# Janspiry/Image-Super-Resolution-via-Iterative-Refinement

Measured on NVIDIA H100. Metric: diffusion steps/sec (batch16, 16->128 SR3), higher is better.
Workload: dtype bf16

## Files before the change

image-super-resolution-via-iterative-refinement_b200/csrc/engine.cu:

```cuda
#include <cuda.h>
#include <cuda_runtime.h>

#include <cmath>
#include <cstdarg>
#include <cstdlib>
#include <cstring>
#include <functional>
#include <limits>
#include <map>
#include <memory>
#include <mutex>
#include <stdexcept>
#include <string>
#include <vector>

#include "../../include/sr3_b200.h"
#include "aux_kernels.cuh"
#include "attn_wgmma.cuh"
#include "train_kernels.cuh"

using namespace sr3;
typedef __nv_bfloat16 bf16;

namespace {
// ... 81 lines not shown
    long long b_rows = 0; int b_K = 0;
    std::vector<KSlab> slabs;
    int block_n = 128;
    int w_box = 16, h_box = 8, b_box = 1;
    int mh = 1;
    int pingpong = 0;
    int tall = 0;
    int a_box_w = 0, a_box_h = 0, a_box_b = 0;
    int a_half_off = 0;
    bool b_is_param = false;
    int ksplit_max = 1;
    int tiles_w = 1, tiles_h = 1, tiles_b = 1, n_tiles = 1, nz = 1;
    int a_zstep = 0, b_zrows = 0;
    int z_phase = 0; long long z_off_hi = 0, z_off_lo = 0;
    int passes = 1, lo_b_col = 0, lo_a_chan[2] = {0, 0};
    long long lo_out_off = 0, lo_t_off = 0;
    int mode = 0, OW = 0, OH = 1, OB = 1, n_valid = 0;
    int out_imgs = 0;
    float scale = 1.f;
    const float* bias = nullptr; const float* bias2 = nullptr; int bias2_stride = 0;
    const float* resid = nullptr; OutSpec rs{};
    float* out_f32 = nullptr; OutSpec os{};
    bf16* out_bf16 = nullptr; OutSpec hs{};
    bf16* out_t = nullptr; int t_col0 = 0, t_rows = 0, t_ld = 0, t_per = 1;
    double* stats = nullptr; int stats_C = 0, stats_coff = 0;
    const StepCtl* ctl = nullptr; PostParams post{};
};

OutSpec nhwc_out(int H, int W, int C, long long off = 0) {
    OutSpec s; s.sZ = 0; s.sB = 1LL * H * W * C; s.sH = 1LL * W * C; s.sW = C; s.off = off; return s;
}

constexpr int SMEM_LIMIT = 232448;
int pick_stages(int block_n, int a_stage_bytes, int b_taps, bool resid, int num_k) {
    int s = GEMM_MAX_STAGES;
    if (const char* e = getenv("SR3_STAGES")) s = atoi(e);
    if (s > GEMM_MAX_STAGES) s = GEMM_MAX_STAGES;
    while (s > 1 && gemm_smem_bytes(block_n, a_stage_bytes, b_taps, s, resid, num_k) > SMEM_LIMIT) --s;
    if (s < 1) s = 1;
    return s;
}
int current_device() { int dev = 0; CK(cudaGetDevice(&dev)); return dev; }
int num_sms() {
    static std::map<int, int> cache;
    static std::mutex mu;
    std::lock_guard<std::mutex> lock(mu);
    const int dev = current_device();
    auto it = cache.find(dev);
    if (it != cache.end()) return it->second;
    int n = 0;
    CK(cudaDeviceGetAttribute(&n, cudaDevAttrMultiProcessorCount, dev));
    cache[dev] = n;
    return n;
}
bool first_use_on_device(std::vector<int>& seen) {
    static std::mutex mu;
    std::lock_guard<std::mutex> lock(mu);
    const int dev = current_device();
    for (int d : seen) if (d == dev) return false;
    seen.push_back(dev);
    return true;
}
template <typename... KArgs, typename... Args>
void launch_k(void (*kernel)(KArgs...), dim3 grid, dim3 block, size_t smem, cudaStream_t st, Args&&... args) {
    cudaLaunchConfig_t cfg{};
    cfg.gridDim = grid; cfg.blockDim = block; cfg.dynamicSmemBytes = smem; cfg.stream = st;
    cudaLaunchAttribute attr[1];
    attr[0].id = cudaLaunchAttributeProgrammaticStreamSerialization;
    attr[0].val.programmaticStreamSerializationAllowed = 1;
    cfg.attrs = attr; cfg.numAttrs = 1;
    CK(cudaLaunchKernelEx(&cfg, kernel, std::forward<Args>(args)...));
// ... 197 lines not shown
        if (d.out_f32 && d.resid) REQUIRE(zo == zr, "output and residual must share the batch coordinate");
        if (!d.out_f32) p.out_map = p.res_map;
        if (!d.resid) p.res_map = p.out_map;
        p.epi_c4_is_z = (d.out_f32 ? zo : zr) ? 1 : 0;
    } else {
        p.out_map = p.b_map; p.res_map = p.b_map;
    }
    p.ksplit = 1;
    {
        const int tiles = d.tiles_w * d.tiles_h * d.tiles_b * d.n_tiles * d.nz;
        const int ks = d.ksplit_max;
        if (ks > 1 && !d.pingpong && d.mode == 0 && d.out_f32 && d.block_n >= 32 && d.n_valid % 32 == 0) {
            int want = num_sms() / tiles;
            if (want > ks) want = ks;
            if (want > p.num_k * d.passes / 2) want = p.num_k * d.passes / 2;
            const int units = d.mh * (d.block_n / 32) * 4;
            if (want > units) want = units;
            want = fit_split(want, tiles);
            if (want > 1) {
                p.ksplit = want;
                p.ws = static_cast<float*>(mem.alloc((size_t)tiles * want * d.mh * 128 * d.block_n * sizeof(float), false));
                p.counters = static_cast<unsigned int*>(mem.alloc((size_t)tiles * sizeof(unsigned int)));
            }
        }
    }
    const int total_tiles = d.tiles_w * d.tiles_h * d.tiles_b * d.n_tiles * d.nz * p.ksplit;
    int ctas = total_tiles < num_sms() ? total_tiles : num_sms();
    if (const char* e = getenv("SR3_MAX_CTAS")) { int v = atoi(e); if (v > 0 && v < ctas) ctas = v; }
    REQUIRE(p.ksplit == 1 || ctas == total_tiles, "split-K launch needs one CTA per (tile, split) pair: %d CTAs for %d (SR3_MAX_CTAS with a split tile)", ctas, total_tiles);
    const dim3 grid(ctas, 1, 1);
    const int bn = d.block_n;
    const int mh = d.mh;
    const bool res_smem = p.tma_epi && d.resid != nullptr && p.ksplit <= 1;
    p.stages = pick_stages(d.block_n, p.a_stage_bytes, p.b_taps, res_smem, p.num_k);
    const int smem = gemm_smem_bytes(bn, p.a_stage_bytes, p.b_taps, p.stages, res_smem, p.num_k);
    REQUIRE(smem <= SMEM_LIMIT, "gemm shared memory %d exceeds the limit", smem);
    init_gemm_attrs();
    REQUIRE((bn == 16 || bn == 32 || bn == 64 || bn == 128 || bn == 256) && (mh == 1 || (mh == 2 && bn <= 128 && bn != 32)), "unsupported tile %dx%d", 128 * mh, bn);
    const bool pp = d.pingpong != 0;
    REQUIRE(!pp || (gemm_pingpong_ok(bn, mh) && p.ksplit == 1 && d.mode == 0), "no ping-pong form of tile %dx%d (split %d)", 128 * mh, bn, p.ksplit);
    if (geo) {
        geo->tall = d.tall; geo->mh = mh; geo->block_n = bn; geo->h_box = d.h_box; geo->b_box = d.b_box;
        geo->ksplit = p.ksplit; geo->stages = p.stages; geo->ctas = ctas; geo->tiles = total_tiles / p.ksplit; geo->res_smem = res_smem ? 1 : 0;
    }
    if (schedule) *schedule = pp ? 1 : 0;
    std::shared_ptr<GemmParams> sp = std::make_shared<GemmParams>(p);
    if (g_gemm_registry) {
        GemmHandle h; h.p = sp; h.w_ptr = d.b_ptr; h.w_bytes = 2LL * d.b_rows * d.b_K; h.w_is_param = d.b_is_param; h.bn = bn; h.mh = mh;
        g_gemm_registry->push_back(h);
    }
    return [sp, grid, bn, mh, pp, smem](cudaStream_t st) {
        const GemmParams& p = *sp;
        if (pp) {
            if (mh == 2) launch_gemm_bn<64, 2, true>(p, grid, smem, st);
            else if (bn == 64) launch_gemm_bn<64, 1, true>(p, grid, smem, st);
            else launch_gemm_bn<128, 1, true>(p, grid, smem, st);
            return;
        }
        switch (bn) {
            case 16: if (mh == 2) launch_gemm_bn<16, 2>(p, grid, smem, st); else launch_gemm_bn<16, 1>(p, grid, smem, st); break;
            case 32: launch_gemm_bn<32, 1>(p, grid, smem, st); break;
            case 64: if (mh == 2) launch_gemm_bn<64, 2>(p, grid, smem, st); else launch_gemm_bn<64, 1>(p, grid, smem, st); break;
            case 128: if (mh == 2) launch_gemm_bn<128, 2>(p, grid, smem, st); else launch_gemm_bn<128, 1>(p, grid, smem, st); break;
            default: launch_gemm_bn<256, 1>(p, grid, smem, st); break;
        }
    };
}

// ... 103 lines not shown
                    const double cpp = model(tiles, nstage * npass, stage_bytes, c.mh * 128, c.bn, sp1, true);
                    if (cpp < best_pp) { best_pp = cpp; pp_mh = c.mh; pp_bn = c.bn; }
                }
                if (c.bn == 128 && has_resid && sp <= 1) continue;
                if (cost < best) { best = cost; mh = c.mh; bn = c.bn; split = sp; }
            }
            if (!shape_forced && pp_bn && (pp_force || (pp_auto && best_pp < best))) { mh = pp_mh; bn = pp_bn; split = 1; pp = 1; }
        }
        if (const char* e = getenv("SR3_TALL_BN")) { int v = atoi(e); if ((v == 32 || v == 64 || v == 128) && cout % v == 0) { bn = v; split = 16; } }
        if (const char* e = getenv("SR3_TALL_MH")) { int v = atoi(e); if (v == 1 || v == 2) { mh = v; split = 16; } }
        if (mh == 2 && bn == 32) bn = 64;
        if (shape_forced) pp = (pp_force && gemm_pingpong_ok(bn, mh)) ? 1 : 0;
        if (pp) split = 1;
        d.mh = mh; d.block_n = bn; d.ksplit_max = split; d.pingpong = pp;
        geom(mh, d.h_box, d.b_box);
        d.a_box_w = 8; d.a_box_b = d.b_box;
        if (mh == 2 && d.b_box == 1) { d.a_box_h = 34; d.a_half_off = 16 * 1024; }
        else if (mh == 2) { d.a_box_h = 18; d.a_half_off = 18 * 1024; }
        else { d.a_box_h = 18; d.a_half_off = 0; }
    } else {
        d.tall = 0; d.mh = 1;
        pick_image_box(OW, OH, d.w_box, d.h_box, d.b_box);
        d.block_n = pick_block_n(cout);
        const long long mt = (long long)(OW / d.w_box) * ((OH + d.h_box - 1) / d.h_box) * ((Bt + d.b_box - 1) / d.b_box) * nz;
        if (getenv("SR3_BLOCK_N") == nullptr && cout % 32 == 0) {
            const int nstage = (((int)d.slabs.size() + 2) / 3) * npass;
            double best = 1e300, best_pp = 1e300;
            int pp_bn = 0;
            for (int bn = 128; bn >= 32; bn >>= 1) {
                if (cout % bn != 0) continue;
                int sp = 1;
                const long long tiles = mt * (cout / bn);
                const double cost = model(tiles, nstage, 3ll * (16384 + bn * 128), 128, bn, sp);
                if (gemm_pingpong_ok(bn, 1) && gemm_smem_bytes(bn, 3 * 16384, 3, 2, has_resid, nstage / npass) <= SMEM_LIMIT) {
                    int sp1 = 1;
                    const double cpp = model(tiles, nstage, 3ll * (16384 + bn * 128), 128, bn, sp1, true);
                    if (cpp < best_pp) { best_pp = cpp; pp_bn = bn; }
                }
                if (bn == 128 && sp > 1) continue;
                if (cost < best) { best = cost; d.block_n = bn; d.ksplit_max = sp; }
            }
            if (pp_bn && (pp_force || (pp_auto && best_pp < best))) { d.block_n = pp_bn; d.ksplit_max = 1; d.pingpong = 1; }
        } else if (pp_force && gemm_pingpong_ok(d.block_n, 1)) {
            d.pingpong = 1;
        }
    }
    if (d.pingpong) d.ksplit_max = 1;
    if (const char* e = getenv("SR3_KSPLIT")) d.ksplit_max = atoi(e);
    d.tiles_w = OW / d.w_box; d.tiles_h = (OH + d.h_box - 1) / d.h_box; d.tiles_b = (Bt + d.b_box - 1) / d.b_box;
}

void pick_image_box(int W, int H, int& w_box, int& h_box, int& b_box) {
    w_box = W < 16 ? W : 16;
    h_box = 128 / w_box;
    if (h_box > H) h_box = H;
    if (w_box * h_box < 32) h_box = 32 / w_box;
    b_box = 128 / (w_box * h_box);
}

int pick_block_n(int cout) {
    if (const char* e = getenv("SR3_BLOCK_N")) { int v = atoi(e); if (v == 32 || v == 64 || v == 128 || v == 256) if (cout % v == 0) return v; }
    if (cout % 128 == 0) return 128;
    if (cout % 64 == 0) return 64;
    return 16;
}

void add_conv_slabs(std::vector<KSlab>& slabs, int a_sel, int cin, int ksize, int stride, int b_col0, int row = 0) {
// ... 2034 lines not shown
```

image-super-resolution-via-iterative-refinement_b200/csrc/gemm_wgmma.cuh:

```cuda
#pragma once
#include <cuda.h>
#include <type_traits>
#include "ptx.cuh"

namespace sr3 {

struct OutSpec {
    long long sZ, sB, sH, sW, off;
};

struct StepCtl {
    int t_cur;
    int t_next;
    int nl_from_table;
    int out_mode;
    int use_noise_buf;
    int write_mean;
    int clip;
    int update_state;
    unsigned long long seed;
    unsigned long long sample_offset;
};

struct PostParams {
// ... 18 lines not shown
struct StageDesc {
    int ntaps;
    int a_multi;
    int a_sel;
    int pad0;
    StageTap tap[3];
    int pad1, pad2;
};

struct GemmParams {
    CUtensorMap a_map[2];
    CUtensorMap b_map;
    CUtensorMap out_map;
    CUtensorMap res_map;
    const StageDesc* ktab;
    int num_k;
    int a_stage_bytes;
    int a_box_bytes;
    int a_half_off;
    int b_taps;
    int tiles_w, tiles_h, tiles_b;
    int n_tiles, nz;
    int tma_epi;
    int epi_c4_is_z;
    int ksplit;
    float* ws;
    unsigned int* counters;
    const void* pf_ptr;
    long long pf_bytes;
    int w_box, h_box, b_box;
    int w_shift, h_shift;
    int a_zstep, b_zrows;
    int stages;
    int mode;
    int OW, OH, OB, n_valid;
    float scale;
    const float* bias;
    const float* bias2;
    int bias2_stride;
    const float* resid;
    OutSpec rs;
    float* out_f32;
    OutSpec os;
    __nv_bfloat16* out_bf16;
    OutSpec hs;
    __nv_bfloat16* out_t;
    int t_col0, t_rows, t_ld, t_per;
    double* stats;
    int stats_C, stats_coff;
    const StepCtl* ctl;
    PostParams post;
    int z_phase;
    long long z_off_hi, z_off_lo;
    int passes, lo_b_col, lo_a_chan[2];
    long long lo_out_off, lo_t_off;
};

constexpr int GEMM_THREADS = 288;
constexpr int GEMM_EPI_WARPS = 8;
constexpr int GEMM_PRODUCER_WARP = 8;
constexpr int GEMM_MAX_STAGES = 8;
__host__ __device__ constexpr int gemm_epi_warp_bytes(bool resid) { return resid ? 12288 : 4096; }
__host__ __device__ constexpr int gemm_epi_bytes(bool resid) { return GEMM_EPI_WARPS * gemm_epi_warp_bytes(resid); }
constexpr int GEMM_MAX_K = 160;
constexpr int GEMM_HDR_BYTES = 2048;
__host__ __device__ constexpr bool gemm_single_wg(int block_n, int mh) { return mh == 1 && block_n <= 32; }
__host__ __device__ constexpr bool gemm_pingpong_ok(int block_n, int mh) { return (mh == 2 && block_n == 64) || (mh == 1 && (block_n == 64 || block_n == 128)); }
constexpr int GEMM_ORDER_BAR = 2;
__host__ __device__ constexpr int gemm_stage_readers(int block_n, int mh, bool pp) { return (pp || gemm_single_wg(block_n, mh)) ? 1 : 2; }
__host__ __device__ constexpr int gemm_aux_bytes(int num_k) {
    return GEMM_HDR_BYTES + ((num_k * 96 + 127) / 128) * 128  + GEMM_EPI_WARPS * 2 * 32 * 4 ;
}

__host__ __device__ constexpr int gemm_stage_bytes(int block_n, int a_stage_bytes, int b_taps) { return a_stage_bytes + b_taps * block_n * 128; }
__host__ __device__ constexpr int gemm_smem_bytes(int block_n, int a_stage_bytes, int b_taps, int stages, bool resid, int num_k) {
    return stages * gemm_stage_bytes(block_n, a_stage_bytes, b_taps) + gemm_epi_bytes(resid) + 1024  + gemm_aux_bytes(num_k);
}

__device__ __forceinline__ void philox4x32_10(uint32_t (&c)[4], uint32_t k0, uint32_t k1) {
#pragma unroll
    for (int r = 0; r < 10; ++r) {
        const uint32_t hi0 = __umulhi(0xD2511F53u, c[0]), lo0 = 0xD2511F53u * c[0];
        const uint32_t hi1 = __umulhi(0xCD9E8D57u, c[2]), lo1 = 0xCD9E8D57u * c[2];
        const uint32_t n0 = hi1 ^ c[1] ^ k0, n1 = lo1, n2 = hi0 ^ c[3] ^ k1, n3 = lo0;
        c[0] = n0; c[1] = n1; c[2] = n2; c[3] = n3;
        k0 += 0x9E3779B9u; k1 += 0xBB67AE85u;
    }
}
__device__ __forceinline__ void box_muller(uint32_t a, uint32_t b, float& z0, float& z1) {
    const float u1 = (static_cast<float>(a) + 1.0f) * 2.3283064365386963e-10f;
    const float u2 = static_cast<float>(b) * 2.3283064365386963e-10f;
    const float r = sqrtf(-2.0f * logf(u1));
    float s, c;
    sincospif(2.0f * u2, &s, &c);
    z0 = r * c; z1 = r * s;
}

__device__ __forceinline__ double stats_quantize(double v) { return rint(v * 1048576.0) * (1.0 / 1048576.0); }

__device__ __forceinline__ float warp_column_sums(float (&v)[32]) {
    const uint32_t lane = lane_id();
#pragma unroll
    for (int half = 16; half >= 1; half >>= 1) {
        const bool up = (lane & half) != 0;
#pragma unroll
        for (int j = 0; j < half; ++j) {
            const float keep = up ? v[j + half] : v[j];
            const float send = up ? v[j] : v[j + half];
            v[j] = keep + __shfl_xor_sync(0xffffffffu, send, half);
// ... 23 lines not shown
    if (t > 0) {
        if (ctl.use_noise_buf) {
            for (int c = 0; c < q.C; ++c) z[c] = q.noise_buf[(static_cast<long long>(img) * q.C + c) * plane + pix];
        } else {
            uint32_t ctr[4] = {static_cast<uint32_t>(pix), static_cast<uint32_t>(ctl.sample_offset + img), static_cast<uint32_t>(t),
                               static_cast<uint32_t>((ctl.sample_offset + img) >> 32)};
            philox4x32_10(ctr, static_cast<uint32_t>(ctl.seed), static_cast<uint32_t>(ctl.seed >> 32));
            box_muller(ctr[0], ctr[1], z[0], z[1]);
            box_muller(ctr[2], ctr[3], z[2], z[3]);
        }
    }
    for (int c = 0; c < q.C; ++c) {
        const long long idx = (static_cast<long long>(img) * q.C + c) * plane + pix;
        const float xt = q.x_state[idx];
        float x0 = __fsub_rn(__fmul_rn(c1, xt), __fmul_rn(c2, eps[c]));
        if (ctl.clip) x0 = fminf(fmaxf(x0, -1.0f), 1.0f);
        const float mean = __fadd_rn(__fmul_rn(pc1, x0), __fmul_rn(pc2, xt));
        if (ctl.write_mean) q.mean_out[idx] = mean;
        const float xn = __fadd_rn(mean, __fmul_rn(z[c], sigma));
        if (ctl.update_state) {
            q.x_state[idx] = xn;
            __nv_bfloat16* ib = q.in_buf + (static_cast<long long>(img) * plane + pix) * q.in_C + q.in_coff + c;
            const __nv_bfloat16 hi = __float2bfloat16_rn(xn);
            *ib = hi;
            if (q.in_lo_off) ib[q.in_lo_off] = __float2bfloat16_rn(xn - __bfloat162float(hi));
        }
    }
}

__device__ __forceinline__ void gemm_stage_setup(const GemmParams& p, const GemmParams* pm, const uint32_t base, uint8_t* base_ptr, const int block_n,
                                                 const int mh, const bool pp) {
    const int stages = p.stages;
    const int stage_bytes = p.a_stage_bytes + p.b_taps * block_n * 128;
    const bool use_res_tma = p.tma_epi && p.resid != nullptr && p.ksplit <= 1;
    const int epi_bytes = GEMM_EPI_WARPS * gemm_epi_warp_bytes(use_res_tma);
    uint8_t* aux_ptr = base_ptr + GEMM_HDR_BYTES + stages * stage_bytes + epi_bytes;
    {
        const int4* src = reinterpret_cast<const int4*>(p.ktab);
        int4* dst = reinterpret_cast<int4*>(aux_ptr);
        for (int i = threadIdx.x; i < p.num_k * 6; i += blockDim.x) dst[i] = __ldg(&src[i]);
    }
    if (threadIdx.x == 0) {
        tma_prefetch_desc(&pm->a_map[0]);
        tma_prefetch_desc(&pm->a_map[1]);
        tma_prefetch_desc(&pm->b_map);
        if (p.tma_epi) { tma_prefetch_desc(&pm->out_map); tma_prefetch_desc(&pm->res_map); }
        const uint32_t bar_base = base;
        const uint32_t consumers = gemm_stage_readers(block_n, mh, pp);
        for (int s = 0; s < stages; ++s) {
            mbar_init(bar_base + 8u * s, 1);
            mbar_init(bar_base + 8u * (GEMM_MAX_STAGES + s), consumers);
        }
        for (int w = 0; w < 2 * GEMM_EPI_WARPS; ++w) mbar_init(bar_base + 8u * (2 * GEMM_MAX_STAGES + w), 1);
        fence_mbar_init();
    }
}

template <int WN, int CW, int CL>
__device__ __forceinline__ void acc_chunk_rows(const float (&acc)[2][WN / 2], float* buf, float (&v)[32]) {
    static_assert(CW <= 32 && (CL + 1) * CW <= WN, "accumulator chunk");
    const int lane = static_cast<int>(lane_id());
    __syncwarp();
#pragma unroll
    for (int i = 0; i < 2; ++i) {
#pragma unroll
        for (int j = (CL * CW) / 2; j < ((CL + 1) * CW) / 2; j += 2) {
            const int r = (lane >> 2) + 8 * i + 16 * ((j >> 1) & 1);
            const int cc = 8 * (j >> 2) - CL * CW + 2 * (lane & 3);
            *reinterpret_cast<float2*>(buf + r * 32 + (cc ^ ((r & 7) << 2))) = make_float2(acc[i][j], acc[i][j + 1]);
// ... 36 lines not shown
                }
            }
        }
        clear();
    }
    __device__ __forceinline__ void start(const GemmParams& p, const int im, const int nb0, const int ch0, const int lane) {
        if (im != img || nb0 != n0) { flush(p, ch0, lane); img = im; n0 = nb0; }
    }
    __device__ __forceinline__ void add(const int c, const double s, const double q) {
#pragma unroll
        for (int cc = 0; cc < N; ++cc)
            if (cc == c) { sum[cc] += s; sq[cc] += q; }
    }
};

template <int BLOCK_N, int MH, bool PP = false>
__device__ __forceinline__ void gemm_tile_body(const GemmParams& p, const GemmParams* pm, const uint32_t base, uint8_t* base_ptr,
                                               const int cta, const int ncta) {
    static_assert(!PP || gemm_pingpong_ok(BLOCK_N, MH), "ping-pong tile shape");
    constexpr int B_BYTES = BLOCK_N * 128;
    constexpr bool SINGLE = !PP && gemm_single_wg(BLOCK_N, MH);
    constexpr int WN = (PP || SINGLE || MH == 2) ? BLOCK_N : BLOCK_N / 2;
    constexpr int AH = PP ? MH : 1;
    constexpr int CW = WN < 32 ? WN : 32;
    constexpr int NCH = BLOCK_N >= 32 ? BLOCK_N / 32 : 1;
    constexpr int NITEMS = MH * NCH;
    constexpr int OWN = PP ? NITEMS : SINGLE ? 1 : NITEMS / 2;
    constexpr int NSTAT = PP ? NCH : OWN;
    static_assert(WN % CW == 0 && AH * WN <= 128, "accumulator shape");

    const int stages = p.stages;
    const int stage_bytes = p.a_stage_bytes + p.b_taps * B_BYTES;
    const bool use_res_tma = p.tma_epi && p.resid != nullptr && p.ksplit <= 1;
    const int epi_warp_bytes = gemm_epi_warp_bytes(use_res_tma);
    const int epi_bytes = GEMM_EPI_WARPS * epi_warp_bytes;
    const uint32_t bar_base = base;
    const uint32_t stage_base = base + GEMM_HDR_BYTES;
    uint8_t* stage_ptr = base_ptr + GEMM_HDR_BYTES;
    const uint32_t epi_base = stage_base + stages * stage_bytes;
    auto full_bar = [&](int s) { return bar_base + 8u * s; };
    auto empty_bar = [&](int s) { return bar_base + 8u * (GEMM_MAX_STAGES + s); };
    auto res_bar = [&](int w, int b) { return bar_base + 8u * (2 * GEMM_MAX_STAGES + 2 * w + b); };
    uint8_t* aux_ptr = stage_ptr + stages * stage_bytes + epi_bytes;
    StageDesc* ktab_s = reinterpret_cast<StageDesc*>(aux_ptr);
    float* bias_s = reinterpret_cast<float*>(aux_ptr + ((p.num_k * 96 + 127) / 128) * 128);

    const int warp = threadIdx.x >> 5;
    const int lane = threadIdx.x & 31;
    const int tiles_m = p.tiles_w * p.tiles_h * p.tiles_b;
    const int ksplit = p.ksplit > 1 ? p.ksplit : 1;
    const int total_tiles = tiles_m * p.n_tiles * p.nz * ksplit;
    const int num_kt = p.num_k * (p.passes > 1 ? p.passes : 1);
    gemm_stage_setup(p, pm, base, base_ptr, BLOCK_N, MH, PP);
    __syncthreads();
    if (warp == 2 && lane == 0 && p.pf_bytes > 0) {
        long long chunk = ((p.pf_bytes + ncta - 1) / ncta + 15) & ~15ll;
        const long long off = chunk * cta;
        if (off < p.pf_bytes) {
            if (off + chunk > p.pf_bytes) chunk = (p.pf_bytes - off) & ~15ll;
            const char* src = static_cast<const char*>(p.pf_ptr) + off;
            for (long long done = 0; done < chunk; done += 65536) {
                const unsigned int n = static_cast<unsigned int>(chunk - done < 65536 ? chunk - done : 65536);
                if (n >= 16) asm volatile("cp.async.bulk.prefetch.L2.global [%0], %1;" ::"l"(src + done), "r"(n) : "memory");
            }
        }
    }
    pdl_launch_dependents();
// ... 21 lines not shown
            decode(tile, w0, h0, b0, n0, z);
            const int brow = n0 + z * p.b_zrows;
            const int zdw = p.z_phase ? (z & 1) : 0, zdh = p.z_phase ? (z >> 1) : 0;
            const int sp = tile % ksplit;
            const int k0 = (num_kt * sp) / ksplit, k1 = (num_kt * (sp + 1)) / ksplit;
            for (int k = k0; k < k1; ++k) {
                mbar_wait(empty_bar(s), ph ^ 1u);
                if (elect_one_sync()) {
                    const int pass = k / p.num_k;
                    const StageDesc& e = ktab_s[k - pass * p.num_k];
                    const int a_lo = (pass == 2) ? p.lo_a_chan[e.a_sel] : 0, b_lo = (pass == 1) ? p.lo_b_col : 0;
                    const uint32_t a_dst = stage_base + s * stage_bytes;
                    const int na = e.a_multi ? e.ntaps : 1;
                    mbar_arrive_expect_tx(full_bar(s), na * p.a_box_bytes + e.ntaps * B_BYTES);
                    for (int t = 0; t < na; ++t)
                        tma_load_5d(a_dst + (e.a_multi ? e.tap[t].a_off : 0), &pm->a_map[e.a_sel], full_bar(s), e.tap[t].a_chan + a_lo, w0 + e.tap[t].dw + zdw, e.tap[t].p,
                                    h0 + e.tap[t].dh + (e.a_multi ? zdh : 0), b0);
                    for (int t = 0; t < e.ntaps; ++t)
                        tma_load_2d(a_dst + p.a_stage_bytes + t * B_BYTES, &pm->b_map, full_bar(s), e.tap[t].b_col + b_lo, brow);
                }
                __syncwarp();
                if (++s == stages) { s = 0; ph ^= 1u; }
            }
        }
    } else if (warp < GEMM_EPI_WARPS) {
        const int g = warp >> 2;
        const int q = warp & 3;
        const int ew = warp;
        const bool mma_wg = !SINGLE || g == 0;
        const int own0 = (SINGLE || PP) ? 0 : g * OWN;
        const int ch0 = PP ? 0 : own0 % NCH;
        const int acc_half = (MH == 2 && !PP) ? g : 0;
        const int acc_c0 = (MH == 1 && !SINGLE && !PP) ? g * WN : 0;
        const uint32_t out_smem = epi_base + ew * epi_warp_bytes;
        const uint32_t res_smem = out_smem + 4096;
        uint8_t* out_ptr = stage_ptr + stages * stage_bytes + ew * epi_warp_bytes;
        uint8_t* res_ptr = out_ptr + 4096;
        const bool use_out_tma = p.tma_epi && p.out_f32 != nullptr;
        uint32_t res_phase = 0;
        uint32_t res_count = 0;
        uint32_t bias_slot = 0;
        bool out_pending = false;
        int s = 0;
        uint32_t ph = 0;
        StatRun<NSTAT> st_own;
        for (int tile = tile_begin + (PP ? g : 0); tile < tile_end; tile += (PP ? 2 : 1)) {
            float acc[AH][2][WN / 2];
            int w0, h0, b0, n0, z;
            decode(tile, w0, h0, b0, n0, z);
            if constexpr (PP) {
                const long long pos = static_cast<long long>(tile - tile_begin) * num_kt;
                s = static_cast<int>(pos % stages);
                ph = static_cast<uint32_t>((pos / stages) & 1);
            }
            auto item_geom = [&](int item, int qq, int& half, int& ch, int& sw, int& sh, int& c4) {
                half = item / NCH; ch = item % NCH;
                const int r0 = half * 128 + qq * 32;
                sw = r0 & (p.w_box - 1);
                sh = (r0 >> p.w_shift) & (p.h_box - 1);
                const int sb = r0 >> (p.w_shift + p.h_shift);
                c4 = p.epi_c4_is_z ? z : (b0 + sb);
            };
            auto request_resid = [&](int item) {
                int half, ch, sw, sh, c4;
                item_geom(item, q, half, ch, sw, sh, c4);
                const uint32_t b = res_count & 1;
                mbar_arrive_expect_tx(res_bar(ew, b), 4096);
                tma_load_5d(res_smem + b * 4096, &pm->res_map, res_bar(ew, b), n0 + ch * 32, w0 + sw, 0, h0 + sh, c4);
            };
            auto item_bias = [&](int item, int qq) {
                float bv = 0.f;
                const int half = item / NCH, ch = item % NCH;
                const int img = b0 + ((half * 128 + qq * 32) >> (p.w_shift + p.h_shift));
                const int n = n0 + ch * 32 + lane;
                if (n < p.n_valid) {
                    if (p.bias) bv += __ldg(&p.bias[n]);
                    if (p.bias2) bv += __ldcg(&p.bias2[static_cast<long long>(img < p.OB ? img : 0) * p.bias2_stride + n]);
                }
                return bv;
            };
            constexpr int WJ = MH * 128;
            auto ws_row = [&](int item, int qq) {
                return (static_cast<long long>(item % NCH) * 8 * WJ + (item / NCH) * 128 + qq * 32 + lane) * 4;
            };
            if (use_res_tma && mma_wg && lane == 0) request_resid(own0);
            float bvs[OWN] = {};
            if constexpr (BLOCK_N != 16) {
                if (mma_wg) {
#pragma unroll
                    for (int ii = 0; ii < OWN; ++ii) bvs[ii] = item_bias(own0 + ii, q);
                }
            }
            const int sp = tile % ksplit;
            if (mma_wg) {
                const int k0 = (num_kt * sp) / ksplit, k1 = (num_kt * (sp + 1)) / ksplit;
                int zrow_off = 0;
                if (p.z_phase) {
                    const int zz = (tile / ksplit) / (tiles_m * p.n_tiles);
                    zrow_off = (zz >> 1) * 1024;
                }
                const uint32_t a_base = stage_base + acc_half * p.a_half_off;
                const uint32_t b_base = stage_base + p.a_stage_bytes + acc_c0 * 128;
                const int li = tile - tile_begin;
                if (PP && li > 0) asm volatile("bar.sync %0, 256;" ::"r"(GEMM_ORDER_BAR + g) : "memory");
                int prev = -1;
                for (int k = k0; k < k1; ++k) {
                    mbar_wait(full_bar(s), ph);
                    const StageDesc& e = ktab_s[k % p.num_k];
                    const int ntaps = __shfl_sync(0xffffffffu, e.ntaps, 0);
                    auto issue = [&](auto nt_c) {
                        wgmma_fence();
#pragma unroll
                        for (int t = 0; t < decltype(nt_c)::value; ++t) {
                            const uint32_t a_addr = a_base + s * stage_bytes + e.tap[t].a_off + (e.a_multi ? 0 : zrow_off);
                            const uint32_t b_addr = b_base + s * stage_bytes + t * B_BYTES;
#pragma unroll
                            for (int kk = 0; kk < 4; ++kk) {
                                const uint64_t bdesc = wgmma_desc_sw128(b_addr + kk * 32, 16, 1024);
// ... 52 lines not shown
                            const uint64_t now = globaltimer_ns();
                            if (t0 == 0) t0 = now;
                            if (now - t0 > 4000000000ull) __trap();
                        }
                    }
                    __threadfence();
                }
                __syncwarp();
                asm volatile("bar.sync 1, 256;" ::: "memory");
            }
            const bool to_ws = (!PP && ksplit > 1 && pass == 0);
            auto epi_item = [&](const int item, const int qq, const float bv, const bool last, auto&& fetch, auto&& add_stats) {
                int half, ch, sw, sh, c4;
                item_geom(item, qq, half, ch, sw, sh, c4);
                const int row = half * 128 + qq * 32 + lane;
                const int w = row & (p.w_box - 1);
                const int h = (row >> p.w_shift) & (p.h_box - 1);
                const int bb = row >> (p.w_shift + p.h_shift);
                const int ow = w0 + w, oh = h0 + h, img = b0 + bb;
                const bool row_ok = (ow < p.OW) && (oh < p.OH) && (img < p.OB);
                float v[32];
                if constexpr (BLOCK_N == 16) {
                    fetch(v);
                    if (row_ok) {
                        float eps[4] = {0.f, 0.f, 0.f, 0.f};
                        for (int c = 0; c < p.post.C; ++c) eps[c] = v[c] + __ldg(&p.bias[c]);
                        final_epilogue(p, eps, img, oh, ow);
                    }
                } else {
                    const int nb = n0 + ch * 32;
                    float* bs = bias_s + (ew * 2 + (bias_slot++ & 1u)) * 32;
                    bs[lane] = bv;
                    __syncwarp();
                    if (use_res_tma) {
                        ++res_count;
                        if (!last && lane == 0) request_resid(item + 1);
                    }
                    fetch(v);
                    const float ep_scale = p.scale;
                    const bool full = (nb + 32 <= p.n_valid);
#pragma unroll
                    for (int j4 = 0; j4 < 8; ++j4) {
                        const float4 bq = reinterpret_cast<const float4*>(bs)[j4];
                        const float bb4[4] = {bq.x, bq.y, bq.z, bq.w};
#pragma unroll
                        for (int jj = 0; jj < 4; ++jj) {
                            const int j = 4 * j4 + jj;
                            float x = v[j] * ep_scale + bb4[jj];
                            if (!full && nb + j >= p.n_valid) x = 0.f;
                            v[j] = x;
                        }
                    }
                    if (use_res_tma) {
                        const uint32_t b = (res_count - 1) & 1;
                        mbar_wait(res_bar(ew, b), (res_phase >> b) & 1u);
                        res_phase ^= (1u << b);
                        const uint8_t* rp = res_ptr + b * 4096 + lane * 128;
#pragma unroll
                        for (int j = 0; j < 8; ++j) {
                            const float4 r = *reinterpret_cast<const float4*>(rp + ((j ^ (lane & 7)) << 4));
                            v[4 * j] += r.x; v[4 * j + 1] += r.y; v[4 * j + 2] += r.z; v[4 * j + 3] += r.w;
                        }
                        __syncwarp();
                    } else if (row_ok && p.resid) {
                        const long long ro = out_index(p.rs, z, img, oh, ow);
                        for (int j = 0; j < 32; ++j)
                            if (nb + j < p.n_valid) v[j] += __ldcg(&p.resid[ro + nb + j]);
                    }
                    if (use_out_tma) {
                        if (out_pending) {
                            if (lane == 0) tma_store_wait_read<0>();
                            __syncwarp();
                        }
                        uint8_t* op = out_ptr + lane * 128;
#pragma unroll
                        for (int j = 0; j < 8; ++j)
                            *reinterpret_cast<float4*>(op + ((j ^ (lane & 7)) << 4)) = make_float4(v[4 * j], v[4 * j + 1], v[4 * j + 2], v[4 * j + 3]);
                        fence_proxy_async_smem();
                        __syncwarp();
                        if (lane == 0) {
                            if (p.z_phase) tma_store_5d(&pm->out_map, out_smem, (z & 1) * p.n_valid + nb, w0 + sw, z >> 1, h0 + sh, c4);
                            else tma_store_5d(&pm->out_map, out_smem, nb, w0 + sw, 0, h0 + sh, c4);
                            tma_store_commit();
                        }
                        out_pending = true;
                    } else if (row_ok && p.out_f32) {
                        const long long oo = out_index(p.os, z, img, oh, ow) + (p.z_phase ? (z >> 1) * p.z_off_hi + (z & 1) * p.z_off_lo : 0);
                        if (full) {
                            float4* o4 = reinterpret_cast<float4*>(p.out_f32 + oo + nb);
#pragma unroll
                            for (int j = 0; j < 8; ++j) o4[j] = make_float4(v[4 * j], v[4 * j + 1], v[4 * j + 2], v[4 * j + 3]);
                        } else {
                            for (int j = 0; j < 32; ++j)
                                if (nb + j < p.n_valid) p.out_f32[oo + nb + j] = v[j];
                        }
                    }
                    if (p.out_t && nb >= p.t_col0) {
                        if (ow < p.OW && oh < p.OH && nb + 32 <= p.n_valid) {
                            __nv_bfloat16* tp = p.out_t + (static_cast<long long>(img / p.t_per) * p.t_rows + (nb - p.t_col0)) * p.t_ld +
                                                (img % p.t_per) * (p.OH * p.OW) + oh * p.OW + ow;
#pragma unroll
                            for (int j = 0; j < 32; ++j) {
                                const __nv_bfloat16 hi = __float2bfloat16_rn(v[j]);
                                tp[static_cast<long long>(j) * p.t_ld] = hi;
                                if (p.lo_t_off) tp[static_cast<long long>(j) * p.t_ld + p.lo_t_off] = __float2bfloat16_rn(v[j] - __bfloat162float(hi));
                            }
                        }
                    } else if (row_ok && p.out_bf16) {
                        const long long ho = out_index(p.hs, z, img, oh, ow);
                        if (full) {
                            uint4* o4 = reinterpret_cast<uint4*>(p.out_bf16 + ho + nb);
#pragma unroll
                            for (int j = 0; j < 4; ++j) {
                                __nv_bfloat162 h0v = __floats2bfloat162_rn(v[8 * j], v[8 * j + 1]);
                                __nv_bfloat162 h1v = __floats2bfloat162_rn(v[8 * j + 2], v[8 * j + 3]);
// ... 4 lines not shown
                                uu.z = *reinterpret_cast<uint32_t*>(&h2v); uu.w = *reinterpret_cast<uint32_t*>(&h3v);
                                o4[j] = uu;
                            }
                        } else {
                            for (int j = 0; j < 32; ++j)
                                if (nb + j < p.n_valid) p.out_bf16[ho + nb + j] = __float2bfloat16_rn(v[j]);
                        }
                        if (p.lo_out_off) {
                            __nv_bfloat16* lp = p.out_bf16 + ho + nb + p.lo_out_off;
                            if (full) {
                                uint4* o4 = reinterpret_cast<uint4*>(lp);
#pragma unroll
                                for (int j = 0; j < 4; ++j) {
                                    float r[8];
#pragma unroll
                                    for (int u = 0; u < 8; ++u) r[u] = v[8 * j + u] - __bfloat162float(__float2bfloat16_rn(v[8 * j + u]));
                                    __nv_bfloat162 h0v = __floats2bfloat162_rn(r[0], r[1]), h1v = __floats2bfloat162_rn(r[2], r[3]);
                                    __nv_bfloat162 h2v = __floats2bfloat162_rn(r[4], r[5]), h3v = __floats2bfloat162_rn(r[6], r[7]);
                                    uint4 uu;
                                    uu.x = *reinterpret_cast<uint32_t*>(&h0v); uu.y = *reinterpret_cast<uint32_t*>(&h1v);
                                    uu.z = *reinterpret_cast<uint32_t*>(&h2v); uu.w = *reinterpret_cast<uint32_t*>(&h3v);
                                    o4[j] = uu;
                                }
                            } else {
                                for (int j = 0; j < 32; ++j)
                                    if (nb + j < p.n_valid) lp[j] = __float2bfloat16_rn(v[j] - __bfloat162float(__float2bfloat16_rn(v[j])));
                            }
                        }
                    }
                    if (p.stats) {
                        double cs, cq;
                        if (use_out_tma) {
                            const unsigned int okm = __ballot_sync(0xffffffffu, row_ok);
                            const uint8_t* colp = out_ptr + ((lane & 3) << 2);
                            const int cq4 = lane >> 2;
                            const float sft = *reinterpret_cast<const float*>(colp + (cq4 << 4));
                            float a0 = 0.f, a1 = 0.f, q0 = 0.f, q1 = 0.f;
                            if (okm == 0xffffffffu) {
#pragma unroll
                                for (int r = 0; r < 32; r += 2) {
                                    const float x0 = *reinterpret_cast<const float*>(colp + r * 128 + ((cq4 ^ (r & 7)) << 4)) - sft;
                                    const float x1 = *reinterpret_cast<const float*>(colp + (r + 1) * 128 + ((cq4 ^ ((r + 1) & 7)) << 4)) - sft;
                                    a0 += x0; q0 = fmaf(x0, x0, q0);
                                    a1 += x1; q1 = fmaf(x1, x1, q1);
                                }
                            } else {
#pragma unroll
                                for (int r = 0; r < 32; r += 2) {
                                    float x0 = *reinterpret_cast<const float*>(colp + r * 128 + ((cq4 ^ (r & 7)) << 4)) - sft;
                                    float x1 = *reinterpret_cast<const float*>(colp + (r + 1) * 128 + ((cq4 ^ ((r + 1) & 7)) << 4)) - sft;
                                    if (!((okm >> r) & 1u)) x0 = 0.f;
                                    if (!((okm >> (r + 1)) & 1u)) x1 = 0.f;
                                    a0 += x0; q0 = fmaf(x0, x0, q0);
                                    a1 += x1; q1 = fmaf(x1, x1, q1);
                                }
                            }
                            const double n_ok = static_cast<double>(__popc(okm)), ds = static_cast<double>(sft);
                            const double da = static_cast<double>(a0 + a1), dq = static_cast<double>(q0 + q1);
                            cs = da + n_ok * ds;
                            cq = dq + 2.0 * ds * da + n_ok * ds * ds;
                        } else {
                            float s2[32];
#pragma unroll
                            for (int j = 0; j < 32; ++j) {
                                const float x = row_ok ? v[j] : 0.f;
                                v[j] = x; s2[j] = x * x;
                            }
                            cs = static_cast<double>(warp_column_sums(v));
                            cq = static_cast<double>(warp_column_sums(s2));
                        }
                        add_stats(cs, cq);
                    }
                }
            };
            if (pass == 0) {
                if (mma_wg) {
                    if (!PP && p.stats && !to_ws) st_own.start(p, b0 + ((acc_half * 128 + q * 32) >> (p.w_shift + p.h_shift)), n0, ch0, lane);
                    static_for<OWN>([&](auto ii_c) {
                        constexpr int ii = decltype(ii_c)::value;
                        constexpr int AHI = PP ? ii / NCH : 0, ACL = PP ? ii % NCH : ii;
                        if constexpr (PP) {
                            if (ACL == 0 && p.stats) st_own.start(p, b0 + ((AHI * 128 + q * 32) >> (p.w_shift + p.h_shift)), n0, 0, lane);
                        }
                        auto stage_acc = [&](float (&v)[32]) {
                            if (out_pending) {
                                if (lane == 0) tma_store_wait_read<0>();
                                __syncwarp();
                            }
                            acc_chunk_rows<WN, CW, ACL>(acc[AHI], reinterpret_cast<float*>(out_ptr), v);
                        };
                        if (to_ws) {
                            float v[32];
                            stage_acc(v);
                            float4* dst = reinterpret_cast<float4*>(p.ws + static_cast<long long>(tile) * SLICE + ws_row(own0 + ii, q));
#pragma unroll
                            for (int j = 0; j < 8; ++j) __stcg(dst + j * WJ, make_float4(v[4 * j], v[4 * j + 1], v[4 * j + 2], v[4 * j + 3]));
                        } else {
                            epi_item(own0 + ii, q, bvs[ii], ii + 1 == OWN, stage_acc, [&](double cs, double cq) { st_own.add(PP ? ACL : ii, cs, cq); });
                        }
                    });
                }
            } else {
                StatRun<NCH> st_ws;
#pragma unroll 1
                for (int it = sp + ksplit * ew; it < NITEMS * 4; it += ksplit * GEMM_EPI_WARPS) {
                    const int item = it >> 2, qq = it & 3;
                    if (p.stats) st_ws.start(p, b0 + (((item / NCH) * 128 + qq * 32) >> (p.w_shift + p.h_shift)), n0, 0, lane);
                    epi_item(item, qq, BLOCK_N != 16 ? item_bias(item, qq) : 0.f, true,
                             [&](float (&v)[32]) {
                                 const float* src0 = p.ws + static_cast<long long>(tile - sp) * SLICE + ws_row(item, qq);
#pragma unroll
                                 for (int j = 0; j < 32; ++j) v[j] = 0.f;
                                 for (int s2 = 0; s2 < ksplit; ++s2) {
                                     const float4* src = reinterpret_cast<const float4*>(src0 + s2 * SLICE);
#pragma unroll
                                     for (int j = 0; j < 8; ++j) {
                                         const float4 r = __ldcg(src + j * WJ);
                                         v[4 * j] += r.x; v[4 * j + 1] += r.y; v[4 * j + 2] += r.z; v[4 * j + 3] += r.w;
                                     }
                                 }
                             },
                             [&](double cs, double cq) { st_ws.add(item % NCH, cs, cq); });
// ... 20 lines not shown
```

Baseline: 140.2.

## Rotate multiple epilogue smem buffers to overlap TMA stores with next item

Generalizes the per-warp epilogue staging area from a fixed out/residual pair into a rotating ring of 4KB buffers (three when a TMA residual is loaded, two otherwise if that does not cost a pipeline stage). The epilogue now waits for all but one outstanding TMA store instead of draining every store before reusing the staging buffer, so the write-out of one item can overlap processing of the next. Residual prefetches and output stores share the rotating buffers, with added proxy fences. This uses more shared memory and adds buffer-rotation logic, which risks subtle reuse hazards and fewer pipeline stages in some configurations.

```diff
diff --git a/image-super-resolution-via-iterative-refinement_b200/csrc/engine.cu b/image-super-resolution-via-iterative-refinement_b200/csrc/engine.cu
--- a/image-super-resolution-via-iterative-refinement_b200/csrc/engine.cu
+++ b/image-super-resolution-via-iterative-refinement_b200/csrc/engine.cu
@@ -137,11 +137,11 @@
 }
 
 constexpr int SMEM_LIMIT = 232448;
-int pick_stages(int block_n, int a_stage_bytes, int b_taps, bool resid, int num_k) {
+int pick_stages(int block_n, int a_stage_bytes, int b_taps, int epi_bufs, int num_k) {
     int s = GEMM_MAX_STAGES;
     if (const char* e = getenv("SR3_STAGES")) s = atoi(e);
     if (s > GEMM_MAX_STAGES) s = GEMM_MAX_STAGES;
-    while (s > 1 && gemm_smem_bytes(block_n, a_stage_bytes, b_taps, s, resid, num_k) > SMEM_LIMIT) --s;
+    while (s > 1 && gemm_smem_bytes(block_n, a_stage_bytes, b_taps, s, epi_bufs, num_k) > SMEM_LIMIT) --s;
     if (s < 1) s = 1;
     return s;
 }
@@ -405,8 +405,10 @@
     const int bn = d.block_n;
     const int mh = d.mh;
     const bool res_smem = p.tma_epi && d.resid != nullptr && p.ksplit <= 1;
-    p.stages = pick_stages(d.block_n, p.a_stage_bytes, p.b_taps, res_smem, p.num_k);
-    const int smem = gemm_smem_bytes(bn, p.a_stage_bytes, p.b_taps, p.stages, res_smem, p.num_k);
+    p.epi_bufs = res_smem ? 3 : 1;
+    p.stages = pick_stages(d.block_n, p.a_stage_bytes, p.b_taps, p.epi_bufs, p.num_k);
+    if (!res_smem && pick_stages(d.block_n, p.a_stage_bytes, p.b_taps, 2, p.num_k) == p.stages) p.epi_bufs = 2;
+    const int smem = gemm_smem_bytes(bn, p.a_stage_bytes, p.b_taps, p.stages, p.epi_bufs, p.num_k);
     REQUIRE(smem <= SMEM_LIMIT, "gemm shared memory %d exceeds the limit", smem);
     init_gemm_attrs();
     REQUIRE((bn == 16 || bn == 32 || bn == 64 || bn == 128 || bn == 256) && (mh == 1 || (mh == 2 && bn <= 128 && bn != 32)), "unsupported tile %dx%d", 128 * mh, bn);
@@ -576,7 +578,7 @@
                 int sp = 1;
                 const long long tiles = mt * (cout / bn);
                 const double cost = model(tiles, nstage, 3ll * (16384 + bn * 128), 128, bn, sp);
-                if (gemm_pingpong_ok(bn, 1) && gemm_smem_bytes(bn, 3 * 16384, 3, 2, has_resid, nstage / npass) <= SMEM_LIMIT) {
+                if (gemm_pingpong_ok(bn, 1) && gemm_smem_bytes(bn, 3 * 16384, 3, 2, has_resid ? 3 : 1, nstage / npass) <= SMEM_LIMIT) {
                     int sp1 = 1;
                     const double cpp = model(tiles, nstage, 3ll * (16384 + bn * 128), 128, bn, sp1, true);
                     if (cpp < best_pp) { best_pp = cpp; pp_bn = bn; }
diff --git a/image-super-resolution-via-iterative-refinement_b200/csrc/gemm_wgmma.cuh b/image-super-resolution-via-iterative-refinement_b200/csrc/gemm_wgmma.cuh
--- a/image-super-resolution-via-iterative-refinement_b200/csrc/gemm_wgmma.cuh
+++ b/image-super-resolution-via-iterative-refinement_b200/csrc/gemm_wgmma.cuh
@@ -74,6 +74,7 @@
     int w_shift, h_shift;
     int a_zstep, b_zrows;
     int stages;
+    int epi_bufs;
     int mode;
     int OW, OH, OB, n_valid;
     float scale;
@@ -102,8 +103,7 @@
 constexpr int GEMM_EPI_WARPS = 8;
 constexpr int GEMM_PRODUCER_WARP = 8;
 constexpr int GEMM_MAX_STAGES = 8;
-__host__ __device__ constexpr int gemm_epi_warp_bytes(bool resid) { return resid ? 12288 : 4096; }
-__host__ __device__ constexpr int gemm_epi_bytes(bool resid) { return GEMM_EPI_WARPS * gemm_epi_warp_bytes(resid); }
+__host__ __device__ constexpr int gemm_epi_bytes(int bufs) { return GEMM_EPI_WARPS * bufs * 4096; }
 constexpr int GEMM_MAX_K = 160;
 constexpr int GEMM_HDR_BYTES = 2048;
 __host__ __device__ constexpr bool gemm_single_wg(int block_n, int mh) { return mh == 1 && block_n <= 32; }
@@ -115,8 +115,8 @@
 }
 
 __host__ __device__ constexpr int gemm_stage_bytes(int block_n, int a_stage_bytes, int b_taps) { return a_stage_bytes + b_taps * block_n * 128; }
-__host__ __device__ constexpr int gemm_smem_bytes(int block_n, int a_stage_bytes, int b_taps, int stages, bool resid, int num_k) {
-    return stages * gemm_stage_bytes(block_n, a_stage_bytes, b_taps) + gemm_epi_bytes(resid) + 1024  + gemm_aux_bytes(num_k);
+__host__ __device__ constexpr int gemm_smem_bytes(int block_n, int a_stage_bytes, int b_taps, int stages, int epi_bufs, int num_k) {
+    return stages * gemm_stage_bytes(block_n, a_stage_bytes, b_taps) + gemm_epi_bytes(epi_bufs) + 1024  + gemm_aux_bytes(num_k);
 }
 
 __device__ __forceinline__ void philox4x32_10(uint32_t (&c)[4], uint32_t k0, uint32_t k1) {
@@ -206,9 +206,7 @@
                                                  const int mh, const bool pp) {
     const int stages = p.stages;
     const int stage_bytes = p.a_stage_bytes + p.b_taps * block_n * 128;
-    const bool use_res_tma = p.tma_epi && p.resid != nullptr && p.ksplit <= 1;
-    const int epi_bytes = GEMM_EPI_WARPS * gemm_epi_warp_bytes(use_res_tma);
-    uint8_t* aux_ptr = base_ptr + GEMM_HDR_BYTES + stages * stage_bytes + epi_bytes;
+    uint8_t* aux_ptr = base_ptr + GEMM_HDR_BYTES + stages * stage_bytes + gemm_epi_bytes(p.epi_bufs);
     {
         const int4* src = reinterpret_cast<const int4*>(p.ktab);
         int4* dst = reinterpret_cast<int4*>(aux_ptr);
@@ -311,7 +309,8 @@
     const int stages = p.stages;
     const int stage_bytes = p.a_stage_bytes + p.b_taps * B_BYTES;
     const bool use_res_tma = p.tma_epi && p.resid != nullptr && p.ksplit <= 1;
-    const int epi_warp_bytes = gemm_epi_warp_bytes(use_res_tma);
+    const int epi_bufs = p.epi_bufs;
+    const int epi_warp_bytes = epi_bufs * 4096;
     const int epi_bytes = GEMM_EPI_WARPS * epi_warp_bytes;
     const uint32_t bar_base = base;
     const uint32_t stage_base = base + GEMM_HDR_BYTES;
@@ -399,15 +398,26 @@
         const int ch0 = PP ? 0 : own0 % NCH;
         const int acc_half = (MH == 2 && !PP) ? g : 0;
         const int acc_c0 = (MH == 1 && !SINGLE && !PP) ? g * WN : 0;
-        const uint32_t out_smem = epi_base + ew * epi_warp_bytes;
-        const uint32_t res_smem = out_smem + 4096;
-        uint8_t* out_ptr = stage_ptr + stages * stage_bytes + ew * epi_warp_bytes;
-        uint8_t* res_ptr = out_ptr + 4096;
+        const uint32_t epi_smem = epi_base + ew * epi_warp_bytes;
+        uint8_t* epi_ptr = stage_ptr + stages * stage_bytes + ew * epi_warp_bytes;
         const bool use_out_tma = p.tma_epi && p.out_f32 != nullptr;
         uint32_t res_phase = 0;
         uint32_t res_count = 0;
         uint32_t bias_slot = 0;
         bool out_pending = false;
+        int rot = 0;
+        auto epi_buf = [&](int b) { return epi_ptr + b * 4096; };
+        auto next_buf = [&](int b) { return b + 1 == epi_bufs ? 0 : b + 1; };
+        const bool keep_one = epi_bufs - (use_res_tma ? 1 : 0) >= 2;
+        auto wait_store_read = [&]() {
+            if (out_pending) {
+                if (lane == 0) {
+                    if (keep_one) tma_store_wait_read<1>();
+                    else tma_store_wait_read<0>();
+                }
+                __syncwarp();
+            }
+        };
         int s = 0;
         uint32_t ph = 0;
         StatRun<NSTAT> st_own;
@@ -428,12 +438,16 @@
                 const int sb = r0 >> (p.w_shift + p.h_shift);
                 c4 = p.epi_c4_is_z ? z : (b0 + sb);
             };
-            auto request_resid = [&](int item) {
-                int half, ch, sw, sh, c4;
-                item_geom(item, q, half, ch, sw, sh, c4);
-                const uint32_t b = res_count & 1;
-                mbar_arrive_expect_tx(res_bar(ew, b), 4096);
-                tma_load_5d(res_smem + b * 4096, &pm->res_map, res_bar(ew, b), n0 + ch * 32, w0 + sw, 0, h0 + sh, c4);
+            auto request_resid = [&](int item, int buf) {
+                fence_proxy_async_smem();
+                __syncwarp();
+                if (lane == 0) {
+                    int half, ch, sw, sh, c4;
+                    item_geom(item, q, half, ch, sw, sh, c4);
+                    const uint32_t b = res_count & 1;
+                    mbar_arrive_expect_tx(res_bar(ew, b), 4096);
+                    tma_load_5d(epi_smem + buf * 4096, &pm->res_map, res_bar(ew, b), n0 + ch * 32, w0 + sw, 0, h0 + sh, c4);
+                }
             };
             auto item_bias = [&](int item, int qq) {
                 float bv = 0.f;
@@ -450,7 +464,7 @@
             auto ws_row = [&](int item, int qq) {
                 return (static_cast<long long>(item % NCH) * 8 * WJ + (item / NCH) * 128 + qq * 32 + lane) * 4;
             };
-            if (use_res_tma && mma_wg && lane == 0) request_resid(own0);
+            if (use_res_tma && mma_wg) request_resid(own0, next_buf(rot));
             float bvs[OWN] = {};
             if constexpr (BLOCK_N != 16) {
                 if (mma_wg) {
@@ -569,11 +583,12 @@
                     float* bs = bias_s + (ew * 2 + (bias_slot++ & 1u)) * 32;
                     bs[lane] = bv;
                     __syncwarp();
+                    fetch(v);
+                    const int ob = use_res_tma ? next_buf(rot) : rot;
                     if (use_res_tma) {
                         ++res_count;
-                        if (!last && lane == 0) request_resid(item + 1);
+                        if (!last) request_resid(item + 1, rot);
                     }
-                    fetch(v);
                     const float ep_scale = p.scale;
                     const bool full = (nb + 32 <= p.n_valid);
 #pragma unroll
@@ -592,7 +607,7 @@
                         const uint32_t b = (res_count - 1) & 1;
                         mbar_wait(res_bar(ew, b), (res_phase >> b) & 1u);
                         res_phase ^= (1u << b);
-                        const uint8_t* rp = res_ptr + b * 4096 + lane * 128;
+                        const uint8_t* rp = epi_buf(ob) + lane * 128;
 #pragma unroll
                         for (int j = 0; j < 8; ++j) {
                             const float4 r = *reinterpret_cast<const float4*>(rp + ((j ^ (lane & 7)) << 4));
@@ -605,19 +620,17 @@
                             if (nb + j < p.n_valid) v[j] += __ldcg(&p.resid[ro + nb + j]);
                     }
                     if (use_out_tma) {
-                        if (out_pending) {
-                            if (lane == 0) tma_store_wait_read<0>();
-                            __syncwarp();
-                        }
-                        uint8_t* op = out_ptr + lane * 128;
+                        wait_store_read();
+                        uint8_t* op = epi_buf(ob) + lane * 128;
 #pragma unroll
                         for (int j = 0; j < 8; ++j)
                             *reinterpret_cast<float4*>(op + ((j ^ (lane & 7)) << 4)) = make_float4(v[4 * j], v[4 * j + 1], v[4 * j + 2], v[4 * j + 3]);
                         fence_proxy_async_smem();
                         __syncwarp();
                         if (lane == 0) {
-                            if (p.z_phase) tma_store_5d(&pm->out_map, out_smem, (z & 1) * p.n_valid + nb, w0 + sw, z >> 1, h0 + sh, c4);
-                            else tma_store_5d(&pm->out_map, out_smem, nb, w0 + sw, 0, h0 + sh, c4);
+                            const uint32_t os = epi_smem + ob * 4096;
+                            if (p.z_phase) tma_store_5d(&pm->out_map, os, (z & 1) * p.n_valid + nb, w0 + sw, z >> 1, h0 + sh, c4);
+                            else tma_store_5d(&pm->out_map, os, nb, w0 + sw, 0, h0 + sh, c4);
                             tma_store_commit();
                         }
                         out_pending = true;
@@ -688,7 +701,7 @@
                         double cs, cq;
                         if (use_out_tma) {
                             const unsigned int okm = __ballot_sync(0xffffffffu, row_ok);
-                            const uint8_t* colp = out_ptr + ((lane & 3) << 2);
+                            const uint8_t* colp = epi_buf(ob) + ((lane & 3) << 2);
                             const int cq4 = lane >> 2;
                             const float sft = *reinterpret_cast<const float*>(colp + (cq4 << 4));
                             float a0 = 0.f, a1 = 0.f, q0 = 0.f, q1 = 0.f;
@@ -727,6 +740,8 @@
                         }
                         add_stats(cs, cq);
                     }
+                    if (use_res_tma) rot = rot == 0 ? epi_bufs - 1 : rot - 1;
+                    else if (use_out_tma) rot = next_buf(rot);
                 }
             };
             if (pass == 0) {
@@ -739,11 +754,8 @@
                             if (ACL == 0 && p.stats) st_own.start(p, b0 + ((AHI * 128 + q * 32) >> (p.w_shift + p.h_shift)), n0, 0, lane);
                         }
                         auto stage_acc = [&](float (&v)[32]) {
-                            if (out_pending) {
-                                if (lane == 0) tma_store_wait_read<0>();
-                                __syncwarp();
-                            }
-                            acc_chunk_rows<WN, CW, ACL>(acc[AHI], reinterpret_cast<float*>(out_ptr), v);
+                            wait_store_read();
+                            acc_chunk_rows<WN, CW, ACL>(acc[AHI], reinterpret_cast<float*>(epi_buf(rot)), v);
                         };
                         if (to_ws) {
                             float v[32];
```

After: 140.6 (median of 6 runs). No clear change (+0.3%).
